# olsonanl/close_kmers

Measured on AMD Instinct MI355X. Metric: protein residues/s vs 1B-entry kmer image; 1/2/4/8 MI355X, higher is better.
Workload: dtype u64

## Files before the change

close_kmers_amd/csrc/kgx_internal.h:

```cpp
#ifndef KGX_INTERNAL_H
#define KGX_INTERNAL_H

#include <hip/hip_runtime.h>
#include <stdint.h>

#include "kgx.h"
#include "kgx_line_home.h"

namespace kgx {

constexpr int KMER = 8;
constexpr uint64_t CORE = 1280000000ULL;
constexpr uint64_t MAX_ENCODED = 25600000000ULL;
constexpr uint64_t EMPTY_KEY = MAX_ENCODED + 1;
constexpr int RUN_CAP = 40000 - 2;

constexpr int PROBE_WAVES = 4;
constexpr uint32_t HIT_PLANES = KGX_HIT_PLANES, HIT_PACKED16 = KGX_HIT_PACKED16;
constexpr int PROBE_BUCKET = 0;
constexpr int PROBE_KEY_FIRST = 1;
constexpr int PROBE_AUTO = -1;
constexpr int PROBE_LINE = 2;
constexpr int PROBE_LINE8 = 3;
constexpr int PROBE_J_DEFAULT = 2;
// ... 7 lines not shown

__host__ __device__ inline bool packable(const kgx_sig_kmer &e)
{
    return e.which_kmer > MAX_ENCODED ||
           (e.function_index >= -1 && e.function_index <= PACK_FI_MAX && e.otu_index >= -1 &&
            e.otu_index <= PACK_OTU_MAX);
}

__host__ __device__ inline packed_bucket pack_bucket(const kgx_sig_kmer &e)
{
    packed_bucket b;
    if (e.which_kmer > MAX_ENCODED) {
        b.lo = EMPTY_KEY;
        b.hi = 0;
        return b;
    }
    uint32_t wt;
    __builtin_memcpy(&wt, &e.function_wt, 4);
    const uint64_t fi = (uint64_t)(e.function_index + 1), otu = (uint64_t)(e.otu_index + 1);
    b.lo = e.which_kmer | (fi << 35) | ((otu & 0x1FFu) << 55);
    b.hi = (uint64_t)wt | ((uint64_t)e.avg_from_end << 32) | ((otu >> 9) << 48);
    return b;
}

__host__ __device__ inline kgx_sig_kmer unpack_bucket(const packed_bucket &b)
{
    kgx_sig_kmer e;
    e.which_kmer = b.lo & PACK_KEY_MASK;
    e.otu_index = (int32_t)(((b.lo >> 55) & 0x1FFu) | (((b.hi >> 48) & 0xFFFu) << 9)) - 1;
    e.avg_from_end = (uint16_t)(b.hi >> 32);
    e.pad = 0;
    e.function_index = (int32_t)((b.lo >> 35) & 0xFFFFFu) - 1;
    const uint32_t wt = (uint32_t)b.hi;
    __builtin_memcpy(&e.function_wt, &wt, 4);
    if (e.which_kmer > MAX_ENCODED) {
        e.otu_index = 0;
        e.avg_from_end = 0;
        e.function_index = 0;
        e.function_wt = 0.0f;
    }
    return e;
}

__host__ __device__ inline uint64_t filter_hash(uint64_t key)
{
    uint64_t h = key * 0x9E3779B97F4A7C15ull;
    return h ^ (h >> 29);
}
__host__ __device__ inline uint64_t filter_word(uint64_t h, uint32_t log2_words)
{
    return log2_words ? h >> (64 - log2_words) : 0;
}
__host__ __device__ inline uint64_t filter_bits(uint64_t h)
{
    return (1ull << (h & 63)) | (1ull << ((h >> 6) & 63));
}

inline uint64_t mod_magic(uint64_t n) { return n ? (~0ULL) / n : 0; }


size_t plan_workspace_bytes(uint32_t n_seq);
hipError_t launch_plan(const uint64_t *seq_off, uint32_t n_seq, uint64_t n_residues, uint64_t *wbase,
                       uint32_t *tile_seq, uint32_t tile_windows, void *workspace, uint32_t *status,
                       hipStream_t stream);
size_t plan_look_bytes(uint32_t n_seq);
hipError_t launch_plan_one(const uint64_t *seq_off, uint32_t n_seq, uint64_t n_residues, uint64_t *wbase,
                           uint32_t *tile_seq, uint32_t tile_windows, uint64_t max_tiles, uint32_t *status,
                           hipStream_t stream);
hipError_t launch_plan_fused(const uint64_t *seq_off, uint32_t n_seq, uint64_t n_residues, uint64_t *wbase,
                             uint32_t *tile_seq, uint32_t tile_windows, uint64_t max_tiles, void *look,
                             uint32_t *status, hipStream_t stream);

struct ProbeTable {
    const void *buckets;
    uint64_t num_sigs;
    uint32_t home;
    uint64_t magic() const { return mod_magic(num_sigs >> home_shift_of(home)); }
};
hipError_t launch_probe(const uint8_t *residues, uint64_t n_residues, const uint64_t *seq_off,
                        const uint64_t *wbase, const uint32_t *tile_seq, uint32_t n_seq,
                        uint64_t max_tiles, const ProbeTable &t, int layout,
                        const uint64_t *filter, uint32_t filter_log2_words,
                        uint4 *hot, uint4 *cold, uint64_t *hit_mask, int probe_j, int variant,
                        uint32_t lds_kb, uint32_t max_blocks, hipStream_t stream, uint32_t nt_stores = 0);
hipError_t launch_probe_dna(const uint8_t *bases, uint64_t n_bases, const uint64_t *anchor, const uint64_t *wbase,
                            const uint32_t *tile_seq, uint32_t n_seq, uint64_t max_tiles, const ProbeTable &t,
                            uint4 *hot, uint64_t *hit_mask, int probe_j, uint32_t max_blocks,
                            hipStream_t stream);

hipError_t launch_pack(const kgx_sig_kmer *table, packed_bucket *packed, uint64_t n,
                       uint32_t *not_packable, hipStream_t stream);
hipError_t launch_unpack(const packed_bucket *packed, kgx_sig_kmer *out, uint64_t n,
                         hipStream_t stream);
hipError_t launch_filter_build(const void *table, int layout, uint64_t num_sigs, uint64_t *filter,
                               uint32_t log2_words, hipStream_t stream);

enum { SCORE_HYBRID = 0, SCORE_WAVE = 1, SCORE_LANE = 2, SCORE_WAVE_ONLY = 3  };
constexpr uint32_t LONG_SEQ = 2048;
hipError_t launch_score(uint32_t n_seq, uint64_t n_residues, const uint64_t *wbase, const uint32_t *tile_seq,
                        uint64_t max_tiles, const uint64_t *hit_mask, uint32_t tile_windows, uint4 *hot,
                        kgx_call *calls, void *ranges, uint32_t *hit_count, uint32_t *call_count,
                        kgx_params params, uint32_t want, uint32_t hit_format, int variant, uint32_t wave_tiles,
                        const uint32_t *plan_status, hipStream_t stream);
hipError_t launch_best_calls(uint32_t n_seq, const kgx_call *calls, const uint64_t *start, const uint32_t *count,
                             kgx_call *ws, kgx_best_call *out, hipStream_t stream);
hipError_t launch_otus(uint32_t n_seq, const uint64_t *wbase, const uint64_t *hit_mask, uint32_t tile_windows,
                       const uint4 *hot, const uint4 *cold, int32_t *ws, kgx_otu *otus, uint32_t *otu_count,
                       uint32_t hit_format, hipStream_t stream);

constexpr uint32_t SMALL_GATHER_SEQ = 256;
constexpr uint32_t SMALL_COLLECT_BEST_SEQ = 8192;
constexpr uint32_t SMALL_GATHER_BLOCKS = 64;
hipError_t launch_small_gather(uint32_t n, const uint64_t *wbase, const uint64_t *hit_mask, uint32_t tile_windows,
                               const uint32_t *hit_count, const uint32_t *call_count, const uint4 *hot,
                               const uint4 *cold, const kgx_call *calls, const uint32_t *otu_count,
                               const kgx_otu *otus, kgx_hit *hits_out, kgx_call *calls_out, kgx_otu *otus_out,
                               uint64_t *h0, uint64_t *h1, uint64_t *h2, const uint32_t *status,
                               const kgx_best_call *best, kgx_best_call *best_host, uint32_t *status_host,
                               uint64_t *nwin_host, uint32_t *done_host, uint32_t token, uint32_t *blocks_done,
                               uint32_t hit_format, hipStream_t stream);
hipError_t launch_gather(uint32_t n_seq, const uint64_t *wbase, const uint64_t *hit_mask,
                         uint32_t tile_windows, const uint32_t *call_count, const uint4 *hot, const uint4 *cold,
                         const kgx_call *calls, const uint64_t *hit_dense_off,
                         const uint64_t *call_dense_off, kgx_hit *hits_out, kgx_call *calls_out,
                         uint32_t seq_base, uint32_t hit_format, const uint32_t *otu_count, const kgx_otu *otus,
                         const uint64_t *otu_dense_off, kgx_otu *otus_out, hipStream_t stream,
                         uint4 *hits16_out = nullptr,
                         uint32_t *hits12_out = nullptr);
size_t count_scan_workspace_bytes(uint32_t n);
hipError_t launch_count_scan(uint32_t n, const uint32_t *c0, const uint32_t *c1, const uint32_t *c2, uint64_t *o0,
                             uint64_t *o1, uint64_t *o2, void *workspace, hipStream_t stream);
constexpr int SMALL_PIECES = 5;
struct SmallPieces {
    uint4 *dst[SMALL_PIECES];
    const uint4 *src[SMALL_PIECES];
    uint64_t end16[SMALL_PIECES];
};
hipError_t launch_small_upload(const SmallPieces &pc, hipStream_t stream);
hipError_t launch_small_collect(uint32_t n, const uint32_t *c0, const uint32_t *c1, const uint32_t *c2, uint64_t *o0,
                                uint64_t *o1, uint64_t *o2, uint64_t *h0, uint64_t *h1, uint64_t *h2,
                                const uint32_t *status, const uint64_t *wbase, const kgx_best_call *best,
                                kgx_best_call *best_host, uint32_t *status_host, uint64_t *nwin_host,
                                hipStream_t stream);
hipError_t launch_small_collect_best(uint32_t n, const uint32_t *c0, const uint32_t *c1, const uint32_t *c2,
                                     uint64_t *o0, uint64_t *o1, uint64_t *o2, uint64_t *h0, uint64_t *h1,
                                     uint64_t *h2, const uint32_t *status, const uint64_t *wbase,
                                     const kgx_call *calls, const uint32_t *call_count, kgx_call *ws,
                                     kgx_best_call *best, kgx_best_call *best_host, uint32_t *status_host,
                                     uint64_t *nwin_host, hipStream_t stream);
hipError_t launch_copy_counted(void *dst, const void *src, const uint64_t *count, uint64_t cap,
                               uint32_t elem_bytes, int blocks, hipStream_t stream);
hipError_t launch_nul_scan(const uint8_t *d, uint64_t skip, uint64_t n, uint32_t *flag_mapped, hipStream_t stream);

hipError_t launch_copy_to_host(void *dst_mapped, const void *src, uint64_t bytes, int blocks, hipStream_t stream);
struct CopySpans {
    static constexpr int kMax = 8;
    void *dst[kMax];
    const void *src[kMax];
    uint64_t n[kMax];
    bool v16[kMax];
    int count = 0;
    void add(void *d, const void *s, uint64_t bytes)
    {
        if (bytes == 0)
            return;
        if (count == kMax) {
            count = kMax + 1;
            return;
        }
        dst[count] = d;
// ... 65 lines not shown
```

close_kmers_amd/csrc/kgx_probe.hip:

```cpp
#include <algorithm>

#include "kgx_device.h"

namespace kgx {

__device__ __forceinline__ uint3 load_residues(const uint8_t *residues, uint64_t bm, uint64_t n, uint64_t abo)
{
    uint32_t d[3] = {0, 0, 0};
    for (int b = 0; b < 12; b++)
        if (abo + b >= bm && abo + b < bm + n)
            d[b >> 2] |= (uint32_t)residues[abo + b - bm] << (8 * (b & 3));
    return make_uint3(d[0], d[1], d[2]);
}

constexpr int MODE_BUCKET = 0, MODE_KEY_FIRST = 1, MODE_PACKED = 2, MODE_PACKED_KEY_FIRST = 3;

typedef unsigned int u32x4_t __attribute__((ext_vector_type(4)));
template <bool NT> __device__ __forceinline__ uint4 load_record(const uint4 *p)
{
    if (NT) {
        const u32x4_t v = __builtin_nontemporal_load(reinterpret_cast<const u32x4_t *>(p));
        return make_uint4(v.x, v.y, v.z, v.w);
    }
    return *p;
// ... 260 lines not shown
                rec[j].x = m ? pv[j].x : rec[j].x;
                rec[j].y = m ? pv[j].y : rec[j].y;
                rec[j].z = m ? pv[j].z : rec[j].z;
                rec[j].w = m ? pv[j].w : rec[j].w;
            }
            if ((KEY_FIRST || MODE == MODE_PACKED_KEY_FIRST) && m) {
                if (KEY_FIRST)
                    rec[j] = *reinterpret_cast<const uint4 *>(
                        reinterpret_cast<const char *>(table + slot[j]) + 8);
                if (MODE == MODE_PACKED_KEY_FIRST) {
                    const uint64_t hi = packed_w[2 * slot[j] + 1];
                    rec[j] = make_uint4(pv[j].x, pv[j].y, (uint32_t)hi, (uint32_t)(hi >> 32));
                }
            }
            hit[j] = hit[j] || m;
            pend[j] = pend[j] && !m && !stop;
            slot[j] = pend[j] ? (slot[j] + 1 == num_sigs ? 0 : slot[j] + 1) : slot[j];
            more = more || pend[j];
        }
        if (!__any(more))
            break;
    }

    store_tile_hits<J, PACKED>(hit, key, rec, pos, sq, g0, W, lane, hot, cold, hit_mask);
}

__device__ __forceinline__ void probe_slice_aligned(const uint4 *__restrict__ packed, uint32_t n_lines, uint64_t key,
                                                    bool ok, uint32_t home_line, uint32_t q, uint32_t c, uint4 *rec,
                                                    uint8_t *hitf)
{
    constexpr uint32_t G = 4, NQ = 64 / G;
    constexpr uint32_t KEY_HI = (uint32_t)(PACK_KEY_MASK >> 32);
    constexpr uint32_t MAX_HI = (uint32_t)(MAX_ENCODED >> 32), MAX_LO = (uint32_t)MAX_ENCODED;
    static_assert(KEY_HI == 7u && (MARK_BITS_W & KEY_HI) == 0, "key bits 32-34 beside the mark bit");
    const uint32_t own = (uint32_t)(key >> 32) | (uint32_t)ok << 3 | line_mark(key) << 4;
    uint32_t klo[G], kw[G], ln[G];
    uint32_t live = 0;
#pragma unroll
    for (int i = 0; i < (int)G; i++) {
        const int owner = (int)(NQ * i + q);
        klo[i] = (uint32_t)__shfl((int)(uint32_t)key, owner);
        ln[i] = (uint32_t)__shfl((int)home_line, owner);
        const uint32_t o = (uint32_t)__shfl((int)own, owner);
        live |= (o >> 3 & 1u) << i;
        const uint32_t g = o >> 4;
        kw[i] = (o & KEY_HI) | (c == mark_record(g) ? 1u << mark_bit_w(g) : 0u);
    }
    const uint32_t cbit = 1u << c, upto = (2u << c) - 1u;
    constexpr uint32_t MARKED = 1u << G;
    const uint32_t max_lines = n_lines + 2;
    for (uint32_t round = 0;; round++) {
        uint4 d[G];
#pragma unroll
        for (int i = 0; i < (int)G; i++)
            if (live >> i & 1u)
                d[i] = packed[(uint64_t)ln[i] * G + c];
        uint32_t hitm = 0;
#pragma unroll
        for (int i = 0; i < (int)G; i++) {
            const uint32_t kh = d[i].y & KEY_HI;
            const uint32_t diff = (d[i].x ^ klo[i]) | ((d[i].y ^ kw[i]) & KEY_HI);
            const bool ends = diff == 0 || kh > MAX_HI || (kh == MAX_HI && d[i].x > MAX_LO);
            uint32_t w = (ends ? cbit : 0u) | ((d[i].w & kw[i]) >= 1u << 28 ? MARKED : 0u);
            w = live >> i & 1u ? w : 0u;
            w |= (uint32_t)xor_lane((int32_t)w, 1);
            w |= (uint32_t)xor_lane((int32_t)w, 2);
            hitm |= diff == 0 && (w & upto) == cbit ? 1u << i : 0u;
            live = (w & (2u * MARKED - 1)) == MARKED ? live : live & ~(1u << i);
            ln[i] = ln[i] + 1 == n_lines ? 0 : ln[i] + 1;
        }
#pragma unroll
        for (int i = 0; i < (int)G; i++)
            if (hitm >> i & 1u) {
                rec[NQ * i + q] = d[i];
                hitf[NQ * i + q] = 1;
            }
        if (round + 1 >= max_lines)
            live = 0;
        if (!__any(live != 0))
            break;
    }
}

template <int J, int G, bool DNA, bool MARKS, bool TWINS>
__global__ __launch_bounds__(256) void probe_line_kernel(
    const uint8_t *__restrict__ residues, uint64_t n_residues, const uint64_t *__restrict__ seq_off,
    const uint64_t *__restrict__ wbase, const uint32_t *__restrict__ tile_seq, uint32_t n_seq,
    const uint4 *__restrict__ packed, uint64_t num_sigs, uint64_t magic, uint32_t home, uint4 *__restrict__ hot,
    uint4 *__restrict__ cold, uint64_t *__restrict__ hit_mask, uint32_t nt)
{
    constexpr uint32_t T = 64 * J;
    constexpr uint32_t NQ = 64 / G;
    __shared__ uint8_t code_tab[256];
    __shared__ uint8_t cod_tab[DNA ? 68 : 1];
    __shared__ uint4 lds_rec[PROBE_WAVES][T];
    __shared__ uint8_t lds_hit[PROBE_WAVES][T];
    if (DNA) {
        const uint32_t b = threadIdx.x | 0x20u;
        const bool base = b == 'a' || b == 'c' || b == 'g' || b == 't' || b == 'u';
        code_tab[threadIdx.x] = base ? (uint8_t)(((b >> 1) ^ (b >> 2)) & 3u) : (uint8_t)0x40;
        if (threadIdx.x < 65)
            cod_tab[threadIdx.x] = threadIdx.x < 64 ? (uint8_t)residue_code((uint8_t)code11_aa(threadIdx.x)) : 20;
    } else {
        code_tab[threadIdx.x] = (uint8_t)residue_code(threadIdx.x);
    }
    __syncthreads();

    const uint32_t wave = __builtin_amdgcn_readfirstlane(threadIdx.x >> 6);
    const uint32_t lane = lane_id();
    const uint64_t W = wbase[n_seq];
    for (uint64_t tile = (uint64_t)blockIdx.x * PROBE_WAVES + wave; tile * T < W;
         tile += (uint64_t)gridDim.x * PROBE_WAVES) {
    const uint64_t g0 = tile * T;

    uint64_t key[J];
    uint32_t pos[J], sq[J];
    bool ok[J];
    const uint32_t q = lane / G, c = lane % G;
    static_assert(!MARKS || G == 4, "the index's lines are 4 records");
    static_assert(!TWINS || MARKS, "twin records come with marks only");
    if constexpr (MARKS) {
        uint32_t a7[J], b7[J];
        if (DNA)
            encode_tile_dna<J>(residues, n_residues, seq_off, wbase, tile_seq[tile], W, g0, lane, code_tab,
                               cod_tab, key, ok, pos, sq, a7, b7);
        else
            encode_tile<J>(residues, n_residues, seq_off, wbase, tile_seq[tile], W, g0, lane, code_tab, key, ok,
                           pos, sq, a7, b7);
        const uint32_t n_lines = (uint32_t)(num_sigs / G);
        uint32_t home_line[J];
#pragma unroll
        for (int j = 0; j < J; j++) {
            if (TWINS)
                home_line[j] = ok[j] ? (uint32_t)pair_home(a7[j], b7[j], lane, n_lines, magic) : 0;
            else
                home_line[j] = ok[j] ? (uint32_t)line_home_7mers(a7[j], b7[j], n_lines, magic, home_mode_of(home)) : 0;
            lds_hit[wave][64 * j + lane] = 0;
        }
#pragma unroll
        for (int j = 0; j < J; j++)
            probe_slice_aligned(packed, n_lines, key[j], ok[j], home_line[j], q, c, &lds_rec[wave][64 * j],
                                &lds_hit[wave][64 * j]);
    } else {
    if (DNA)
        encode_tile_dna<J>(residues, n_residues, seq_off, wbase, tile_seq[tile], W, g0, lane, code_tab, cod_tab,
                           key, ok, pos, sq);
    else
        encode_tile<J>(residues, n_residues, seq_off, wbase, tile_seq[tile], W, g0, lane, code_tab, key, ok,
                       pos, sq);
    uint64_t first[J];
#pragma unroll
    for (int j = 0; j < J; j++) {
        first[j] = ok[j] ? home_bucket(key[j], num_sigs, magic, home) : 0;
        lds_hit[wave][64 * j + lane] = 0;
    }

    const uint64_t max_lines = num_sigs / G + 2;
#pragma unroll
    for (int j = 0; j < J; j++) {
    uint64_t K[G], cur[G];
    uint32_t live = 0;
    const uint32_t own = (uint32_t)ok[j];
#pragma unroll
    for (int i = 0; i < G; i++) {
        const uint32_t owner = NQ * i + q;
        K[i] = __shfl(key[j], (int)owner);
        cur[i] = __shfl(first[j], (int)owner);
        const uint32_t o = (uint32_t)__shfl((int)own, (int)owner);
        live |= (o & 1u) << i;
    }
    for (uint64_t round = 0;; round++) {
        uint4 d[G];
#pragma unroll
        for (int i = 0; i < G; i++) {
            const uint64_t line = cur[i] - cur[i] % G;
            if ((live >> i & 1u) && line + c < num_sigs)
                d[i] = packed[line + c];
        }
        bool more = false;
#pragma unroll
        for (int i = 0; i < G; i++) {
            const bool act = live >> i & 1u;
            const uint64_t line = cur[i] - cur[i] % G;
            const uint64_t b = line + c;
            const uint64_t kb = ((uint64_t)d[i].y << 32 | d[i].x) & PACK_KEY_MASK;
            const bool valid = act && b < num_sigs && b >= cur[i];
            const uint64_t mm = __ballot(valid && kb == K[i]);
            const uint64_t me = __ballot(valid && kb > MAX_ENCODED);
            const uint32_t gm = (uint32_t)(mm >> (G * q)) & ((1u << G) - 1);
            const uint32_t ge = (uint32_t)(me >> (G * q)) & ((1u << G) - 1);
            if (act) {
                const uint32_t ev = gm | ge;
                if (ev) {
                    const uint32_t first = __builtin_ctz(ev);
                    if (c == first && (gm >> first & 1u)) {
                        const uint32_t w = 64 * j + NQ * i + q;
                        lds_rec[wave][w] = d[i];
                        lds_hit[wave][w] = 1;
                    }
                    live &= ~(1u << i);
                } else if (round + 1 >= max_lines) {
                    live &= ~(1u << i);
                } else {
                    cur[i] = line + G >= num_sigs ? 0 : line + G;
                    more = true;
                }
            }
        }
        if (!__any(more))
            break;
    }
    }
    }
    __builtin_amdgcn_fence(__ATOMIC_RELEASE, "wavefront");
    __builtin_amdgcn_wave_barrier();
    __builtin_amdgcn_fence(__ATOMIC_ACQUIRE, "wavefront");

    bool hit[J];
    uint4 pv[J];
#pragma unroll
    for (int j = 0; j < J; j++) {
        hit[j] = lds_hit[wave][64 * j + lane] != 0;
        pv[j] = hit[j] ? lds_rec[wave][64 * j + lane] : make_uint4(0, 0, 0, 0);
    }
    store_tile_hits<J, true>(hit, key, pv, pos, sq, g0, W, lane, hot, cold, hit_mask, nt != 0);
    }
}

template <int J, int G, bool DNA = false>
static void launch_probe_line(dim3 grid, hipStream_t stream, const uint8_t *residues, uint64_t n_residues,
                              const uint64_t *seq_off, const uint64_t *wbase, const uint32_t *tile_seq,
                              uint32_t n_seq, const ProbeTable &t, uint4 *hot, uint4 *cold, uint64_t *hit_mask,
                              uint32_t dyn_lds, uint32_t nt = 0)
{
    auto *kernel = probe_line_kernel<J, G, DNA, false, false>;
    if constexpr (G == 4)
        if (line_index_aligned(t.num_sigs, t.home))
            kernel = home_twins_of(t.home) ? probe_line_kernel<J, G, DNA, true, true>
                                           : probe_line_kernel<J, G, DNA, true, false>;
    hipLaunchKernelGGL(kernel, grid, dim3(64 * PROBE_WAVES), dyn_lds, stream, residues, n_residues, seq_off, wbase,
                       tile_seq, n_seq, static_cast<const uint4 *>(t.buckets), t.num_sigs, t.magic(), t.home, hot,
                       cold, hit_mask, nt);
}

template <int J, int MODE>
static void launch_probe_m(dim3 grid, hipStream_t stream, const uint8_t *residues, uint64_t n_residues,
                           const uint64_t *seq_off, const uint64_t *wbase, const uint32_t *tile_seq,
                           uint32_t n_seq, const ProbeTable &t, const uint64_t *filter, uint32_t filter_log2,
                           uint4 *hot, uint4 *cold, uint64_t *hit_mask)
{
    if (filter)
        hipLaunchKernelGGL((probe_kernel<J, MODE, true>), grid, dim3(64 * PROBE_WAVES), 0, stream, residues,
                           n_residues, seq_off, wbase, tile_seq, n_seq, t.buckets, t.num_sigs, t.magic(), t.home,
                           filter, filter_log2, hot, cold, hit_mask);
    else
        hipLaunchKernelGGL((probe_kernel<J, MODE, false>), grid, dim3(64 * PROBE_WAVES), 0, stream, residues,
                           n_residues, seq_off, wbase, tile_seq, n_seq, t.buckets, t.num_sigs, t.magic(), t.home,
                           filter, filter_log2, hot, cold, hit_mask);
}

template <int J>
static void launch_probe_j(dim3 grid, hipStream_t stream, int mode, const uint8_t *residues,
                           uint64_t n_residues, const uint64_t *seq_off, const uint64_t *wbase,
                           const uint32_t *tile_seq, uint32_t n_seq, const ProbeTable &t,
                           const uint64_t *filter, uint32_t filter_log2, uint4 *hot, uint4 *cold,
                           uint64_t *hit_mask)
{
#define KGX_PROBE_M(M)                                                                               \
    launch_probe_m<J, M>(grid, stream, residues, n_residues, seq_off, wbase, tile_seq, n_seq, t,     \
                         filter, filter_log2, hot, cold, hit_mask)
    if (mode == MODE_PACKED_KEY_FIRST)
        KGX_PROBE_M(MODE_PACKED_KEY_FIRST);
    else if (mode == MODE_PACKED)
        KGX_PROBE_M(MODE_PACKED);
    else if (mode == MODE_KEY_FIRST)
        KGX_PROBE_M(MODE_KEY_FIRST);
    else
        KGX_PROBE_M(MODE_BUCKET);
#undef KGX_PROBE_M
}

hipError_t launch_probe(const uint8_t *residues, uint64_t n_residues, const uint64_t *seq_off,
                        const uint64_t *wbase, const uint32_t *tile_seq, uint32_t n_seq,
                        uint64_t max_tiles, const ProbeTable &t, int layout,
                        const uint64_t *filter, uint32_t filter_log2,
                        uint4 *hot, uint4 *cold, uint64_t *hit_mask, int probe_j, int variant,
                        uint32_t lds_kb, uint32_t max_blocks, hipStream_t stream, uint32_t nt)
{
    if (max_tiles == 0)
        return hipSuccess;
    if (t.home && layout != KGX_LAYOUT_PACKED16)
        return hipErrorInvalidValue;
    const uint32_t dyn_lds = lds_kb * 1024u > 9216u ? lds_kb * 1024u - 9216u : 0u;
    const dim3 grid((uint32_t)((max_tiles + PROBE_WAVES - 1) / PROBE_WAVES));
    const dim3 lgrid(max_blocks ? std::min<uint32_t>(grid.x, max_blocks) : grid.x);
    if (variant == PROBE_AUTO && layout == KGX_LAYOUT_PACKED16 && !filter)
        variant = PROBE_LINE;
    if ((variant == PROBE_LINE || variant == PROBE_LINE8) && layout == KGX_LAYOUT_PACKED16 && !filter) {
#define KGX_LINE(JJ, GG)                                                                             \
    launch_probe_line<JJ, GG>(lgrid, stream, residues, n_residues, seq_off, wbase, tile_seq, n_seq, t,  \
                              hot, cold, hit_mask, dyn_lds, nt);                                     \
    return hipGetLastError()
        const int key = probe_j * 10 + (variant == PROBE_LINE8 ? 8 : 4);
        switch (key) {
        case 14: KGX_LINE(1, 4);
        case 24: KGX_LINE(2, 4);
        case 34: KGX_LINE(3, 4);
        case 44: KGX_LINE(4, 4);
        case 18: KGX_LINE(1, 8);
        case 28: KGX_LINE(2, 8);
        default: break;
        }
#undef KGX_LINE
    }
    const bool kf = variant == PROBE_AUTO ? layout != KGX_LAYOUT_PACKED16 : variant == PROBE_KEY_FIRST;
    const int mode = layout == KGX_LAYOUT_PACKED16 ? (kf ? MODE_PACKED_KEY_FIRST : MODE_PACKED)
                                                   : (kf ? MODE_KEY_FIRST : MODE_BUCKET);
#define KGX_PROBE_J(JJ)                                                                              \
    launch_probe_j<JJ>(grid, stream, mode, residues, n_residues, seq_off, wbase, tile_seq, n_seq,   \
                       t, filter, filter_log2, hot, cold, hit_mask)
    switch (probe_j) {
    case 1: KGX_PROBE_J(1); break;
    case 2: KGX_PROBE_J(2); break;
    case 3: KGX_PROBE_J(3); break;
    case 4: KGX_PROBE_J(4); break;
    case 5: KGX_PROBE_J(5); break;
    case 8: KGX_PROBE_J(8); break;
    default: return hipErrorInvalidValue;
    }
#undef KGX_PROBE_J
    return hipGetLastError();
}

hipError_t launch_probe_dna(const uint8_t *bases, uint64_t n_bases, const uint64_t *anchor, const uint64_t *wbase,
                            const uint32_t *tile_seq, uint32_t n_seq, uint64_t max_tiles, const ProbeTable &t,
                            uint4 *hot, uint64_t *hit_mask, int probe_j, uint32_t max_blocks,
                            hipStream_t stream)
{
    if (max_tiles == 0)
        return hipSuccess;
    const uint32_t tiles_grid = (uint32_t)((max_tiles + PROBE_WAVES - 1) / PROBE_WAVES);
    const dim3 grid(max_blocks ? std::min<uint32_t>(tiles_grid, max_blocks) : tiles_grid);
#define KGX_DNA(JJ)                                                                                  \
    launch_probe_line<JJ, 4, true>(grid, stream, bases, n_bases, anchor, wbase, tile_seq, n_seq, t,  \
                                   hot, nullptr, hit_mask, 0);                                       \
    return hipGetLastError()
    switch (probe_j) {
    case 1: KGX_DNA(1);
    case 2: KGX_DNA(2);
    case 3: KGX_DNA(3);
    case 4: KGX_DNA(4);
    default: return hipErrorInvalidValue;
    }
#undef KGX_DNA
}

}
```

close_kmers_amd/csrc/kgx_rt.h:

```cpp
#ifndef KGX_RT_H
#define KGX_RT_H

#include <hip/hip_runtime.h>

#include <algorithm>
#include <atomic>
#include <chrono>
#include <condition_variable>
#include <cstdio>
#include <cstdlib>
#include <cstring>
#include <deque>
#include <functional>
#include <memory>
#include <mutex>
#include <string>
#include <thread>
#include <vector>

#include "kgx_internal.h"
#include "kgx_options.h"

namespace kgx {

// ... 271 lines not shown
    explicit operator bool() const { return records != nullptr; }
    uint32_t home_word() const { return kgx::home_word(2u, home, marks, twins); }
};

}

struct kgx_image {
    int device = 0;
    uint64_t num_sigs = 0;
    int layout = KGX_LAYOUT_AOS24;
    kgx_sig_kmer *d_table = nullptr;
    kgx::packed_bucket *d_packed = nullptr;
    kgx::LineIndex lines;
    uint64_t *d_filter = nullptr;
    uint32_t filter_log2_words = 0;
    std::mutex probe_mu;
    hipEvent_t last_probe = nullptr;
    hipStream_t probe_stream = nullptr;
    std::mutex svc_mu;
    std::atomic<kgx::SvcState *> svc{nullptr};
    struct alignas(64) SvcUsers {
        std::atomic<uint32_t> n{0};
    };
    SvcUsers svc_users[32];
    uint32_t svc_slots = 32, svc_idle_us = 1000, svc_life_us = 1000;
    bool svc_configured = false;
    const void *resident() const
    {
        return layout == KGX_LAYOUT_PACKED16 ? static_cast<const void *>(d_packed) : d_table;
    }
    uint64_t resident_bytes() const
    {
        return num_sigs * (layout == KGX_LAYOUT_PACKED16 ? sizeof(kgx::packed_bucket) : sizeof(kgx_sig_kmer));
    }
    kgx::ProbeTable probe_table() const
    {
        return lines ? kgx::ProbeTable{lines.records, 4 * lines.n_lines, lines.home_word()} : reference_table();
    }
    kgx::ProbeTable reference_table() const { return kgx::ProbeTable{resident(), num_sigs, 0u}; }
};

struct kgx_ctx {
    kgx_image *img = nullptr;
    hipStream_t stream = nullptr;
    bool own_stream = false;
    hipEvent_t probe_done = nullptr;
    hipEvent_t probe_ready = nullptr;
    hipStream_t score_stream = nullptr;
    hipEvent_t score_gate = nullptr;
    kgx::DevBuf residues, offsets, wbase, tile_seq, hit_mask, hits, calls, hit_count, call_count,
        dense_hoff, dense_coff, dense_hits, dense_calls, plan_ws, ranges;
    kgx::DevBuf plan_status;
    kgx::DevBuf plan_look;
    kgx::PinnedVec<uint32_t> h_plan_status;
    uint32_t n_seq = 0;
    uint64_t n_residues = 0;
    uint64_t max_tiles = 0;
    uint32_t tile_windows = 64u * kgx::PROBE_J_DEFAULT;
    uint64_t hit_slots = 0;
    const uint64_t *d_off = nullptr;
    bool have_hits = false;
    uint32_t hit_format = kgx::HIT_PLANES;
    bool have_best = false;
    bool defer_best = false;
    kgx::DevBuf best, best_ws, bc_calls, bc_start, bc_count;
    kgx::PinnedVec<kgx_best_call> h_best;
    kgx::DevBuf fq_bases, fq_roff, fq_nfrag, fq_fbase, fq_tmp, fq_res, fq_off, fq_read, fq_frame, fq_start,
        fq_anchor, fq_nres;
    kgx::DevBuf fq_look;
    kgx::PinnedVec<uint64_t> h_fq_tot;
    kgx::FqPending fq_pend;
    struct {
        bool active = false;
        uint32_t n_reads = 0;
        uint64_t n_bases = 0;
    } fq_up;
    kgx::PinnedVec<uint64_t> h_fq_roff;
    kgx::DevBuf fqc_flag, fqc_reads, fqc_nsel, fqc_nfrag, fqc_ncall, fqc_fo, fqc_co, fqc_fc, fqc_len, fqc_coff,
        fqc_calls;
    kgx::PinnedVec<uint32_t> h_fqc_n, h_fqc_reads, h_fqc_fc, h_fqc_len;
    kgx::PinnedVec<uint64_t> h_fqc_tot, h_fqc_fo, h_fqc_coff;
    kgx::PinnedVec<kgx_call> h_fqc_calls;
    kgx::CtxOptions opt;
    std::vector<uint64_t> h_hoff, h_coff, h_ooff;
    kgx::PinnedVec<kgx_hit> h_hits;
    kgx::PinnedVec<kgx_call> h_calls;
    kgx::PinnedVec<kgx_otu> h_otus;
    kgx::PinnedVec<uint32_t> h_ocount;
    kgx::DevBuf otu_ws, otus, otu_count, dense_ooff, dense_otus;
    bool have_otus = false;
    kgx::PinnedVec<uint32_t> h_hcount, h_ccount;
    kgx::PinnedVec<char> h_res;
    kgx_ctx *twin = nullptr;
    kgx::PinnedVec<uint64_t> h_off_stage, h_dense_hoff, h_dense_coff, h_dense_ooff, h_nwin;
    std::unique_ptr<kgx::HostPool> pool;
    std::unique_ptr<kgx::HostPool> stage_pool;
    kgx::PinnedVec<uint4> h_hits16;
    kgx::PinnedVec<uint64_t> h_mask;
    std::vector<uint64_t> h_wstart;
    std::vector<hipEvent_t> chunk_done;
    std::vector<hipEvent_t> chunk_counts;
    std::vector<hipEvent_t> chunk_gathered;
    hipStream_t copy_stream = nullptr;
    hipStream_t up_stream = nullptr;
    kgx::DevBuf up_res, up_off;
    kgx::DevBuf dense_mask, dense_best;
    double rate_hits = 0.35, rate_calls = 0.05, rate_otus = 0.05;
    uint64_t stream_fallbacks = 0;
    bool one_pass_pinned = false;
    uint64_t pinned_batches = 0, nul_reruns = 0;
    uint32_t counts_enqueued = 0;
    kgx::PinnedVec<uint32_t> h_nul;
    std::vector<hipEvent_t> chunk_h2d;
    kgx::DevBuf dense_counts, cscan_ws;
    kgx::PinnedVec<uint32_t> h_counts;
    kgx::PinnedVec<uint32_t> h_hits12;
    kgx::PinnedVec<char> h_res_all;
    kgx::PinnedVec<uint64_t> h_off_all;
    kgx::PinnedVec<uint4> h_small;
    kgx::PinnedVec<uint32_t> h_done;
    kgx::DevBuf small_blocks_done;
    uint64_t fused_batches = 0, small_batches = 0;
    kgx::PinnedVec<uint64_t> h_fwb;
    kgx::PinnedVec<kgx_hit> h_fhits;
    kgx::PinnedVec<kgx_call> h_fcalls;
    kgx::PinnedVec<uint32_t> h_fcounts, h_fdone;
    kgx::PinnedVec<uint64_t> h_fdbg;
    uint32_t small_token = 0;
    kgx::PinnedVec<kgx_call> h_calls_region;
    kgx::PinnedVec<kgx_otu> h_otus_region;
    int compact_out = 0;
    struct CompactSeg {
        uint32_t s0, s1, words;
        uint64_t hit_begin, rec_at, mask_at;
    };
    std::vector<CompactSeg> compact_segs;
    std::vector<kgx_hit_chunk> compact_chunks;
    std::vector<hipEvent_t> prof_ev;
    std::vector<hipEvent_t> prof_done;
    kgx_host_profile last_profile{};
    std::unique_ptr<kgx::RollupScratch> rollup;
};

namespace kgx {
static_assert(CtxOptions{}.probe_variant == PROBE_AUTO && CtxOptions{}.probe_j == PROBE_J_DEFAULT,
              "kgx_options.h spells these two defaults as numbers");
inline void drop_line_index(kgx_image *img)
{
    if (img->lines)
        (void)hipFree(img->lines.records);
    img->lines = LineIndex{};
}
inline bool ctx_lines(const kgx_ctx *c) { return c->img->lines && c->opt.line_index; }
inline ProbeTable ctx_probe_table(const kgx_ctx *c)
{
    return ctx_lines(c) ? c->img->probe_table() : c->img->reference_table();
}
inline void fill_result(kgx_ctx *c, uint32_t n_seq, bool need_hits, bool want_best, uint64_t nwin, kgx_result *out)
{
    out->best = want_best ? c->h_best.data() : nullptr;
    out->n_seq = n_seq;
    out->hit_offsets = c->h_hoff.data();
    out->hits = need_hits ? c->h_hits.data() : nullptr;
    out->call_offsets = c->h_coff.data();
    out->calls = c->h_calls.data();
    out->otu_offsets = c->h_ooff.data();
// ... 28 lines not shown
```

close_kmers_amd/csrc/kgx_runtime.cpp:

```cpp
#include <hip/hip_runtime.h>
#include <sched.h>

#include <algorithm>
#include <cerrno>
#include <ctime>
#include <chrono>
#include <cstdio>
#include <cstdlib>
#include <cstring>
#include <map>
#include <stdexcept>
#include <string>
#include <atomic>
#include <fcntl.h>
#include <mutex>
#include <sys/stat.h>
#include <thread>
#include <unistd.h>
#include <vector>

#include "kgx_rt.h"

using namespace kgx;

// ... 771 lines not shown
    return KGX_OK;
}

int kgx_image_set_layout(kgx_image *img, int layout)
{
    if (!img)
        return fail(KGX_EINVAL, "null image");
    const auto hold = svc_shutdown_hold(img);
    if (layout == KGX_LAYOUT_PACKED16)
        return image_pack(img);
    if (layout == KGX_LAYOUT_AOS24) {
        if (img->lines) {
            HIP_TRY(hipSetDevice(img->device));
            HIP_TRY(hipDeviceSynchronize());
            drop_line_index(img);
        }
        return image_unpack(img);
    }
    return fail(KGX_EINVAL, "unknown layout " + std::to_string(layout));
}

static int image_read(const kgx_image *img, uint64_t first, uint64_t count, kgx_sig_kmer *dst)
{
    HIP_TRY(hipSetDevice(img->device));
    if (img->layout == KGX_LAYOUT_AOS24) {
        HIP_TRY(hipMemcpy(dst, img->d_table + first, count * sizeof(kgx_sig_kmer), hipMemcpyDeviceToHost));
        return KGX_OK;
    }
    const uint64_t slice = 1ull << 24;
    kgx_sig_kmer *tmp = nullptr;
    HIP_TRY(hipMalloc(&tmp, std::max<uint64_t>(1, std::min(slice, count)) * sizeof(kgx_sig_kmer)));
    hipError_t e = hipSuccess;
    for (uint64_t b = 0; b < count && e == hipSuccess; b += slice) {
        const uint64_t m = std::min(slice, count - b);
        e = launch_unpack(img->d_packed + first + b, tmp, m, nullptr);
        if (e == hipSuccess)
            e = hipMemcpy(dst + b, tmp, m * sizeof(kgx_sig_kmer), hipMemcpyDeviceToHost);
    }
    (void)hipFree(tmp);
    if (e != hipSuccess)
        return fail(KGX_EDEVICE, std::string("download: ") + hipGetErrorString(e));
    return KGX_OK;
}

int kgx_image_download(const kgx_image *img, void *dst, uint64_t nbytes)
{
    if (!img || !dst || nbytes != img->num_sigs * sizeof(kgx_sig_kmer))
        return fail(KGX_EINVAL, "bad download buffer");
    return image_read(img, 0, img->num_sigs, static_cast<kgx_sig_kmer *>(dst));
}

int kgx_image_save(const kgx_image *img, const char *dir)
{
    if (!img || !dir)
        return fail(KGX_EINVAL, "null argument");
    const std::string path = std::string(dir) + "/kmer.table.mem_map";
    FILE *f = std::fopen(path.c_str(), "wb");
    if (!f)
        return fail(KGX_EIO, "could not open " + path + " for writing: " + std::strerror(errno));
    const kgx_image_header h{img->num_sigs, sizeof(kgx_sig_kmer), 1};
    bool ok = std::fwrite(&h, sizeof(h), 1, f) == 1;
    const uint64_t chunk = 1ull << 25;
    std::vector<kgx_sig_kmer> buf(std::min(chunk, std::max<uint64_t>(img->num_sigs, 1)));
    for (uint64_t b = 0; ok && b < img->num_sigs; b += chunk) {
        const uint64_t m = std::min(chunk, img->num_sigs - b);
        int rc = image_read(img, b, m, buf.data());
        if (rc) {
            std::fclose(f);
            return rc;
        }
        ok = std::fwrite(buf.data(), sizeof(kgx_sig_kmer), m, f) == m;
    }
    if (std::fclose(f) != 0)
        ok = false;
    return ok ? KGX_OK : fail(KGX_EIO, "short write to " + path);
}


int kgx_ctx_create(kgx_image *img, kgx_ctx **out)
{
    if (!img || !out)
        return fail(KGX_EINVAL, "null argument");
    HIP_TRY(hipSetDevice(img->device));
    kgx_ctx *c = new kgx_ctx;
    c->img = img;
    hipError_t e = hipStreamCreateWithFlags(&c->stream, hipStreamNonBlocking);
    if (e != hipSuccess) {
        delete c;
        return fail(KGX_EDEVICE, std::string("stream: ") + hipGetErrorString(e));
    }
    c->own_stream = true;
    if (const char *sb = std::getenv("KGX_SMALL_BATCH"))
        c->opt.small_batch = std::min<int64_t>(1 << 24, std::max<int64_t>(0, std::atoll(sb)));
    e = hipEventCreateWithFlags(&c->probe_done, hipEventDisableTiming);
    if (e != hipSuccess) {
        (void)hipStreamDestroy(c->stream);
        delete c;
        return fail(KGX_EDEVICE, std::string("event: ") + hipGetErrorString(e));
    }
    *out = c;
    return KGX_OK;
}

int kgx_ctx_destroy(kgx_ctx *c)
{
    if (!c)
        return KGX_OK;
    (void)hipSetDevice(c->img->device);
    if (c->twin)
        kgx_ctx_destroy(c->twin);
    (void)hipStreamSynchronize(c->stream);
    for (DevBuf *b : {&c->residues, &c->offsets, &c->wbase, &c->tile_seq, &c->hit_mask,
                      &c->hits, &c->calls, &c->hit_count, &c->call_count, &c->dense_hoff,
                      &c->dense_coff, &c->dense_hits, &c->dense_calls, &c->plan_ws, &c->ranges})
        b->release();
    {
        std::lock_guard<std::mutex> lock(c->img->probe_mu);
        if (c->img->last_probe == c->probe_done)
            c->img->last_probe = nullptr;
    }
    (void)hipEventDestroy(c->probe_done);
    if (c->probe_ready)
        (void)hipEventDestroy(c->probe_ready);
    if (c->score_gate)
        (void)hipEventDestroy(c->score_gate);
    c->pool.reset();
    c->stage_pool.reset();
    for (hipEvent_t e : c->chunk_done)
        (void)hipEventDestroy(e);
    for (hipEvent_t e : c->chunk_counts)
        (void)hipEventDestroy(e);
    for (hipEvent_t e : c->chunk_gathered)
        (void)hipEventDestroy(e);
    for (hipEvent_t e : c->chunk_h2d)
        (void)hipEventDestroy(e);
    for (hipEvent_t e : c->prof_ev)
        (void)hipEventDestroy(e);
    for (hipEvent_t e : c->prof_done)
        (void)hipEventDestroy(e);
    if (c->copy_stream) {
        (void)hipStreamSynchronize(c->copy_stream);
        (void)hipStreamDestroy(c->copy_stream);
    }
    if (c->up_stream) {
        (void)hipStreamSynchronize(c->up_stream);
        (void)hipStreamDestroy(c->up_stream);
    }
    if (c->own_stream)
        (void)hipStreamDestroy(c->stream);
    delete c;
    return KGX_OK;
}

void *kgx_ctx_stream(kgx_ctx *c) { return c ? (void *)c->stream : nullptr; }

int kgx_ctx_set_stream(kgx_ctx *c, void *stream)
{
    if (!c)
        return fail(KGX_EINVAL, "null ctx");
    if (stream) {
        if (c->own_stream)
            (void)hipStreamDestroy(c->stream);
        c->stream = (hipStream_t)stream;
        c->own_stream = false;
    } else if (!c->own_stream) {
        HIP_TRY(hipStreamCreateWithFlags(&c->stream, hipStreamNonBlocking));
        c->own_stream = true;
    }
// ... 98 lines not shown
    c->have_otus = false;
    return KGX_OK;
}

}

namespace {

uint32_t probe_max_blocks(const kgx_ctx *c)
{
    if (!c->opt.probe_persist)
        return 0;
    int cus = 0;
    if (hipDeviceGetAttribute(&cus, hipDeviceAttributeMultiprocessorCount, c->img->device) != hipSuccess || cus <= 0)
        cus = 256;
    return (uint32_t)c->opt.probe_persist * (uint32_t)cus;
}

template <class Launch>
int probe_chained(kgx_ctx *c, Launch launch)
{
    HIP_TRY(hipSetDevice(c->img->device));
    if (c->img->num_sigs >= (1ull << 40))
        return fail(KGX_ERANGE, "image too large");
    kgx_image *img = c->img;
    std::unique_lock<std::mutex> lock(img->probe_mu, std::defer_lock);
    if (c->opt.probe_serialize && c->opt.probe_stream) {
        lock.lock();
        if (!img->probe_stream)
            HIP_TRY(hipStreamCreateWithFlags(&img->probe_stream, hipStreamNonBlocking));
        if (!c->probe_ready)
            HIP_TRY(hipEventCreateWithFlags(&c->probe_ready, hipEventDisableTiming));
        HIP_TRY(hipEventRecord(c->probe_ready, c->stream));
        HIP_TRY(hipStreamWaitEvent(img->probe_stream, c->probe_ready, 0));
        hipStream_t own = c->stream;
        c->stream = img->probe_stream;
        const hipError_t le = launch();
        c->stream = own;
        HIP_TRY(le);
        HIP_TRY(hipEventRecord(c->probe_done, img->probe_stream));
        HIP_TRY(hipStreamWaitEvent(c->stream, c->probe_done, 0));
        img->last_probe = c->probe_done;
    } else {
        if (c->opt.probe_serialize) {
            lock.lock();
            if (img->last_probe && img->last_probe != c->probe_done)
                HIP_TRY(hipStreamWaitEvent(c->stream, img->last_probe, 0));
        }
        HIP_TRY(launch());
        if (c->opt.probe_serialize) {
            HIP_TRY(hipEventRecord(c->probe_done, c->stream));
            img->last_probe = c->probe_done;
        }
    }
    c->hit_format = c->img->layout == KGX_LAYOUT_PACKED16 ? HIT_PACKED16 : HIT_PLANES;
    c->have_hits = true;
    return KGX_OK;
}

}

namespace kgx {

bool probe_takes_dna(const kgx_ctx *c)
{
    return c->img->layout == KGX_LAYOUT_PACKED16 && !(c->opt.probe_filter && c->img->d_filter) &&
           (c->opt.probe_variant == PROBE_AUTO || c->opt.probe_variant == PROBE_LINE) && c->opt.probe_j >= 1 && c->opt.probe_j <= 4;
}

int stage_probe_dna(kgx_ctx *c, const uint8_t *bases, uint64_t n_bases, const uint64_t *anchors,
                    const uint64_t *d_off)
{
    if ((!anchors || !bases) && c->n_seq)
        return fail(KGX_EINVAL, "fq probe: anchors or bases missing");
    if (d_off != c->d_off)
        return fail(KGX_EINVAL, "fq probe: offsets differ from the plan");
    if (!probe_takes_dna(c) || (int)(c->tile_windows / 64) != c->opt.probe_j)
        return fail(KGX_EINVAL, "fq probe: fragments without residues need the line probe on a PACKED16 image "
                                "(set fq_residues 1 for other probes)");
    return probe_chained(c, [&] {
        return launch_probe_dna(bases, n_bases, anchors, c->wbase.as<uint64_t>(), c->tile_seq.as<uint32_t>(),
                                c->n_seq, c->max_tiles, ctx_probe_table(c),
                                c->hits.as<uint4>(), c->hit_mask.as<uint64_t>(), (int)(c->tile_windows / 64),
                                probe_max_blocks(c), c->stream);
    });
}

}

extern "C" {

int kgx_stage_probe(kgx_ctx *c, const uint8_t *d_res, const uint64_t *d_off)
{
    if (!c || (!d_res && c->n_residues) || d_off != c->d_off)
        return fail(KGX_EINVAL, "probe: residues missing or offsets differ from the plan");
    return probe_chained(c, [&] {
        return launch_probe(d_res, c->n_residues, d_off, c->wbase.as<uint64_t>(), c->tile_seq.as<uint32_t>(),
                            c->n_seq, c->max_tiles, ctx_probe_table(c), c->img->layout,
                            c->opt.probe_filter ? c->img->d_filter : nullptr, c->img->filter_log2_words,
                            c->hits.as<uint4>(), c->hits.as<uint4>() + c->hit_slots, c->hit_mask.as<uint64_t>(),
                            (int)(c->tile_windows / 64), c->opt.probe_variant, (uint32_t)c->opt.probe_lds_kb,
                            probe_max_blocks(c), c->stream, (uint32_t)c->opt.probe_nt);
    });
}



int kgx_stage_score(kgx_ctx *c, const kgx_params *params, uint32_t want)
{
    if (!c)
        return fail(KGX_EINVAL, "null ctx");
    kgx_params p;
    if (params)
        p = *params;
    else
        kgx_params_default(&p);
    HIP_TRY(hipSetDevice(c->img->device));
    const bool best = (want & KGX_WANT_BEST) != 0;
    HIP_TRY(launch_score(c->n_seq, c->n_residues, c->wbase.as<uint64_t>(), c->tile_seq.as<uint32_t>(), c->max_tiles,
                         c->hit_mask.as<uint64_t>(), c->tile_windows, c->hits.as<uint4>(), c->calls.as<kgx_call>(),
                         c->ranges.p, c->hit_count.as<uint32_t>(), c->call_count.as<uint32_t>(), p,
                         want | (best ? KGX_WANT_CALLS : 0u), c->hit_format, c->opt.score_variant,
                         (uint32_t)c->opt.score_wave_tiles, c->plan_status.as<uint32_t>(), c->stream));
    c->have_best = false;
    c->have_otus = false;
    if (want & KGX_WANT_OTU) {
        HIP_TRY(c->otu_ws.reserve(std::max<uint64_t>(c->hit_slots, 1) * sizeof(int32_t)));
        HIP_TRY(c->otus.reserve(std::max<uint64_t>(c->hit_slots, 1) * sizeof(kgx_otu)));
        HIP_TRY(c->otu_count.reserve(std::max<uint64_t>(c->n_seq, 1) * sizeof(uint32_t)));
        HIP_TRY(launch_otus(c->n_seq, c->wbase.as<uint64_t>(), c->hit_mask.as<uint64_t>(), c->tile_windows,
                            c->hits.as<uint4>(), c->hits.as<uint4>() + c->hit_slots, c->otu_ws.as<int32_t>(),
                            c->otus.as<kgx_otu>(), c->otu_count.as<uint32_t>(), c->hit_format, c->stream));
        c->have_otus = true;
    }
    if (best) {
        HIP_TRY(c->best.reserve(std::max<uint64_t>(c->n_seq, 1) * sizeof(kgx_best_call)));
        HIP_TRY(c->best_ws.reserve(c->hit_slots * sizeof(kgx_call)));
        if (!c->defer_best)
            HIP_TRY(launch_best_calls(c->n_seq, c->calls.as<kgx_call>(), c->wbase.as<uint64_t>(),
                                      c->call_count.as<uint32_t>(), c->best_ws.as<kgx_call>(),
                                      c->best.as<kgx_best_call>(), c->stream));
        c->have_best = true;
    }
    return KGX_OK;
}

int kgx_find_best_calls(kgx_ctx *c, const kgx_call *calls, const uint64_t *call_offsets, uint32_t n_seq,
                        kgx_best_call *out)
{
    if (!c || (n_seq && (!call_offsets || !out)))
        return fail(KGX_EINVAL, "null argument");
    if (n_seq == 0)
        return KGX_OK;
    const uint64_t c0 = call_offsets[0], n = call_offsets[n_seq] - c0;
    if (n && !calls)
        return fail(KGX_EINVAL, "null calls");
    std::vector<uint64_t> start(n_seq);
    std::vector<uint32_t> count(n_seq);
    for (uint32_t s = 0; s < n_seq; s++) {
        if (call_offsets[s + 1] < call_offsets[s])
            return fail(KGX_EINVAL, "call_offsets not monotone");
        start[s] = call_offsets[s] - c0;
        count[s] = (uint32_t)(call_offsets[s + 1] - call_offsets[s]);
    }
    HIP_TRY(hipSetDevice(c->img->device));
    HIP_TRY(c->bc_calls.reserve(std::max<uint64_t>(n, 1) * sizeof(kgx_call)));
    HIP_TRY(c->best_ws.reserve(std::max<uint64_t>(n, 1) * sizeof(kgx_call)));
    HIP_TRY(c->bc_start.reserve(n_seq * sizeof(uint64_t)));
    HIP_TRY(c->bc_count.reserve(n_seq * sizeof(uint32_t)));
    HIP_TRY(c->best.reserve(n_seq * sizeof(kgx_best_call)));
    c->have_best = false;
    if (n)
        HIP_TRY(hipMemcpyAsync(c->bc_calls.p, calls + c0, n * sizeof(kgx_call), hipMemcpyHostToDevice, c->stream));
    HIP_TRY(hipMemcpyAsync(c->bc_start.p, start.data(), n_seq * sizeof(uint64_t), hipMemcpyHostToDevice, c->stream));
    HIP_TRY(hipMemcpyAsync(c->bc_count.p, count.data(), n_seq * sizeof(uint32_t), hipMemcpyHostToDevice, c->stream));
    HIP_TRY(launch_best_calls(n_seq, c->bc_calls.as<kgx_call>(), c->bc_start.as<uint64_t>(),
                              c->bc_count.as<uint32_t>(), c->best_ws.as<kgx_call>(), c->best.as<kgx_best_call>(),
                              c->stream));
    HIP_TRY(hipMemcpyAsync(out, c->best.p, n_seq * sizeof(kgx_best_call), hipMemcpyDeviceToHost, c->stream));
    HIP_TRY(hipStreamSynchronize(c->stream));
    return KGX_OK;
}

int kgx_device_result_get(kgx_ctx *c, kgx_device_result *out)
{
// ... 360 lines not shown
```

Baseline: 58.94 billion.

## Defer multi-round line probes into a compacted per-wave list

Adds a deferred probe mode for the aligned G=4 line kernel. It does the first line round for every window slice, then compacts the windows still open into a per-wave LDS list. It then runs the later rounds over that list, 16 keys at a time, so lanes stay busy instead of idling while a few slices chain through many lines. This costs extra LDS (open list and stashed key state), a wave barrier, and more bookkeeping. The mode is on by default, and the environment variable KGX_PROBE_DEFER can switch it off.

```diff
diff --git a/close_kmers_amd/csrc/kgx_internal.h b/close_kmers_amd/csrc/kgx_internal.h
--- a/close_kmers_amd/csrc/kgx_internal.h
+++ b/close_kmers_amd/csrc/kgx_internal.h
@@ -113,10 +113,11 @@
                         uint64_t max_tiles, const ProbeTable &t, int layout,
                         const uint64_t *filter, uint32_t filter_log2_words,
                         uint4 *hot, uint4 *cold, uint64_t *hit_mask, int probe_j, int variant,
-                        uint32_t lds_kb, uint32_t max_blocks, hipStream_t stream, uint32_t nt_stores = 0);
+                        uint32_t lds_kb, uint32_t max_blocks, bool defer, hipStream_t stream,
+                        uint32_t nt_stores = 0);
 hipError_t launch_probe_dna(const uint8_t *bases, uint64_t n_bases, const uint64_t *anchor, const uint64_t *wbase,
                             const uint32_t *tile_seq, uint32_t n_seq, uint64_t max_tiles, const ProbeTable &t,
-                            uint4 *hot, uint64_t *hit_mask, int probe_j, uint32_t max_blocks,
+                            uint4 *hot, uint64_t *hit_mask, int probe_j, uint32_t max_blocks, bool defer,
                             hipStream_t stream);
 
 hipError_t launch_pack(const kgx_sig_kmer *table, packed_bucket *packed, uint64_t n,
diff --git a/close_kmers_amd/csrc/kgx_probe.hip b/close_kmers_amd/csrc/kgx_probe.hip
--- a/close_kmers_amd/csrc/kgx_probe.hip
+++ b/close_kmers_amd/csrc/kgx_probe.hip
@@ -366,7 +366,100 @@
     }
 }
 
-template <int J, int G, bool DNA, bool MARKS, bool TWINS>
+__device__ __forceinline__ uint32_t quad_line_word(const uint4 &d, uint32_t klo, uint32_t kw, bool open,
+                                                   uint32_t cbit, uint32_t &diff)
+{
+    constexpr uint32_t KEY_HI = (uint32_t)(PACK_KEY_MASK >> 32), MARKED = 1u << 4;
+    constexpr uint32_t MAX_HI = (uint32_t)(MAX_ENCODED >> 32), MAX_LO = (uint32_t)MAX_ENCODED;
+    const uint32_t kh = d.y & KEY_HI;
+    diff = (d.x ^ klo) | ((d.y ^ kw) & KEY_HI);
+    const bool ends = diff == 0 || kh > MAX_HI || (kh == MAX_HI && d.x > MAX_LO);
+    uint32_t w = (ends ? cbit : 0u) | ((d.w & kw) >= 1u << 28 ? MARKED : 0u);
+    w = open ? w : 0u;
+    w |= (uint32_t)xor_lane((int32_t)w, 1);
+    w |= (uint32_t)xor_lane((int32_t)w, 2);
+    return w;
+}
+
+__device__ __forceinline__ uint32_t probe_slice_round0(const uint4 *__restrict__ packed, uint64_t key, uint32_t own,
+                                                       uint32_t home_line, uint32_t q, uint32_t c, uint4 *rec,
+                                                       uint8_t *hitf)
+{
+    constexpr uint32_t G = 4, NQ = 64 / G, MARKED = 1u << G;
+    constexpr uint32_t KEY_HI = (uint32_t)(PACK_KEY_MASK >> 32);
+    uint32_t klo[G], kw[G], ln[G];
+    uint32_t live = 0;
+#pragma unroll
+    for (int i = 0; i < (int)G; i++) {
+        const int owner = (int)(NQ * i + q);
+        klo[i] = (uint32_t)__shfl((int)(uint32_t)key, owner);
+        ln[i] = (uint32_t)__shfl((int)home_line, owner);
+        const uint32_t o = (uint32_t)__shfl((int)own, owner);
+        live |= (o >> 3 & 1u) << i;
+        const uint32_t g = o >> 4;
+        kw[i] = (o & KEY_HI) | (c == mark_record(g) ? 1u << mark_bit_w(g) : 0u);
+    }
+    const uint32_t cbit = 1u << c, upto = (2u << c) - 1u;
+    uint4 d[G];
+#pragma unroll
+    for (int i = 0; i < (int)G; i++)
+        if (live >> i & 1u)
+            d[i] = packed[(uint64_t)ln[i] * G + c];
+    uint32_t hitm = 0;
+#pragma unroll
+    for (int i = 0; i < (int)G; i++) {
+        uint32_t diff;
+        const uint32_t w = quad_line_word(d[i], klo[i], kw[i], live >> i & 1u, cbit, diff);
+        hitm |= diff == 0 && (w & upto) == cbit ? 1u << i : 0u;
+        live = (w & (2u * MARKED - 1)) == MARKED ? live : live & ~(1u << i);
+    }
+#pragma unroll
+    for (int i = 0; i < (int)G; i++)
+        if (hitm >> i & 1u) {
+            rec[NQ * i + q] = d[i];
+            hitf[NQ * i + q] = 1;
+        }
+    return live;
+}
+
+__device__ __forceinline__ void probe_tile_deferred(const uint4 *__restrict__ packed, uint32_t n_lines,
+                                                    uint32_t n_open, const uint8_t *list, uint32_t q, uint32_t c,
+                                                    uint4 *rec, uint8_t *hitf)
+{
+    constexpr uint32_t G = 4, NQ = 64 / G, MARKED = 1u << G;
+    constexpr uint32_t KEY_HI = (uint32_t)(PACK_KEY_MASK >> 32);
+    const uint32_t cbit = 1u << c, upto = (2u << c) - 1u;
+    const uint32_t max_lines = n_lines + 2;
+    for (uint32_t p = 0; p < n_open; p += NQ) {
+        bool live = p + q < n_open;
+        uint32_t w = 0;
+        uint4 e = make_uint4(0, 0, 0, 0);
+        if (live) {
+            w = list[p + q];
+            e = rec[w];
+        }
+        const uint32_t klo = e.x, g = e.y >> 4;
+        const uint32_t kw = (e.y & KEY_HI) | (c == mark_record(g) ? 1u << mark_bit_w(g) : 0u);
+        uint32_t ln = e.z;
+        for (uint32_t round = 1;; round++) {
+            uint4 d;
+            if (live)
+                d = packed[(uint64_t)ln * G + c];
+            uint32_t diff;
+            const uint32_t lw = quad_line_word(d, klo, kw, live, cbit, diff);
+            if (diff == 0 && (lw & upto) == cbit) {
+                rec[w] = d;
+                hitf[w] = 1;
+            }
+            live = live && (lw & (2u * MARKED - 1)) == MARKED && round + 1 < max_lines;
+            ln = ln + 1 == n_lines ? 0 : ln + 1;
+            if (!__any(live))
+                break;
+        }
+    }
+}
+
+template <int J, int G, bool DNA, bool MARKS, bool TWINS, bool DEFER>
 __global__ __launch_bounds__(256) void probe_line_kernel(
     const uint8_t *__restrict__ residues, uint64_t n_residues, const uint64_t *__restrict__ seq_off,
     const uint64_t *__restrict__ wbase, const uint32_t *__restrict__ tile_seq, uint32_t n_seq,
@@ -379,6 +472,8 @@
     __shared__ uint8_t cod_tab[DNA ? 68 : 1];
     __shared__ uint4 lds_rec[PROBE_WAVES][T];
     __shared__ uint8_t lds_hit[PROBE_WAVES][T];
+    __shared__ uint8_t lds_open[PROBE_WAVES][DEFER ? T : 1];
+    static_assert(T <= 256, "a window slot is a byte of lds_open");
     if (DNA) {
         const uint32_t b = threadIdx.x | 0x20u;
         const bool base = b == 'a' || b == 'c' || b == 'g' || b == 't' || b == 'u';
@@ -421,10 +516,33 @@
                 home_line[j] = ok[j] ? (uint32_t)line_home_7mers(a7[j], b7[j], n_lines, magic, home_mode_of(home)) : 0;
             lds_hit[wave][64 * j + lane] = 0;
         }
+        if constexpr (DEFER) {
+            uint32_t n_open = 0;
+#pragma unroll
+            for (int j = 0; j < J; j++) {
+                const uint32_t own = (uint32_t)(key[j] >> 32) | (uint32_t)ok[j] << 3 | line_mark(key[j]) << 4;
+                const uint32_t live = probe_slice_round0(packed, key[j], own, home_line[j], q, c,
+                                                         &lds_rec[wave][64 * j], &lds_hit[wave][64 * j]);
+                const uint32_t of_quad = (uint32_t)__shfl((int)live, (int)(G * (lane % NQ)));
+                const bool open = of_quad >> (lane / NQ) & 1u;
+                const uint64_t m = __ballot(open);
+                if (open) {
+                    const uint32_t next = home_line[j] + 1 == n_lines ? 0 : home_line[j] + 1;
+                    lds_rec[wave][64 * j + lane] = make_uint4((uint32_t)key[j], own, next, 0);
+                    lds_open[wave][n_open + lanes_below(m)] = (uint8_t)(64 * j + lane);
+                }
+                n_open += (uint32_t)__popcll(m);
+            }
+            __builtin_amdgcn_fence(__ATOMIC_RELEASE, "wavefront");
+            __builtin_amdgcn_wave_barrier();
+            __builtin_amdgcn_fence(__ATOMIC_ACQUIRE, "wavefront");
+            probe_tile_deferred(packed, n_lines, n_open, lds_open[wave], q, c, lds_rec[wave], lds_hit[wave]);
+        } else {
 #pragma unroll
         for (int j = 0; j < J; j++)
             probe_slice_aligned(packed, n_lines, key[j], ok[j], home_line[j], q, c, &lds_rec[wave][64 * j],
                                 &lds_hit[wave][64 * j]);
+        }
     } else {
     if (DNA)
         encode_tile_dna<J>(residues, n_residues, seq_off, wbase, tile_seq[tile], W, g0, lane, code_tab, cod_tab,
@@ -515,13 +633,18 @@
 static void launch_probe_line(dim3 grid, hipStream_t stream, const uint8_t *residues, uint64_t n_residues,
                               const uint64_t *seq_off, const uint64_t *wbase, const uint32_t *tile_seq,
                               uint32_t n_seq, const ProbeTable &t, uint4 *hot, uint4 *cold, uint64_t *hit_mask,
-                              uint32_t dyn_lds, uint32_t nt = 0)
-{
-    auto *kernel = probe_line_kernel<J, G, DNA, false, false>;
+                              uint32_t dyn_lds, bool defer, uint32_t nt = 0)
+{
+    auto *kernel = probe_line_kernel<J, G, DNA, false, false, false>;
     if constexpr (G == 4)
-        if (line_index_aligned(t.num_sigs, t.home))
-            kernel = home_twins_of(t.home) ? probe_line_kernel<J, G, DNA, true, true>
-                                           : probe_line_kernel<J, G, DNA, true, false>;
+        if (line_index_aligned(t.num_sigs, t.home)) {
+            if (defer)
+                kernel = home_twins_of(t.home) ? probe_line_kernel<J, G, DNA, true, true, true>
+                                               : probe_line_kernel<J, G, DNA, true, false, true>;
+            else
+                kernel = home_twins_of(t.home) ? probe_line_kernel<J, G, DNA, true, true, false>
+                                               : probe_line_kernel<J, G, DNA, true, false, false>;
+        }
     hipLaunchKernelGGL(kernel, grid, dim3(64 * PROBE_WAVES), dyn_lds, stream, residues, n_residues, seq_off, wbase,
                        tile_seq, n_seq, static_cast<const uint4 *>(t.buckets), t.num_sigs, t.magic(), t.home, hot,
                        cold, hit_mask, nt);
@@ -569,13 +692,14 @@
                         uint64_t max_tiles, const ProbeTable &t, int layout,
                         const uint64_t *filter, uint32_t filter_log2,
                         uint4 *hot, uint4 *cold, uint64_t *hit_mask, int probe_j, int variant,
-                        uint32_t lds_kb, uint32_t max_blocks, hipStream_t stream, uint32_t nt)
+                        uint32_t lds_kb, uint32_t max_blocks, bool defer, hipStream_t stream, uint32_t nt)
 {
     if (max_tiles == 0)
         return hipSuccess;
     if (t.home && layout != KGX_LAYOUT_PACKED16)
         return hipErrorInvalidValue;
-    const uint32_t dyn_lds = lds_kb * 1024u > 9216u ? lds_kb * 1024u - 9216u : 0u;
+    const uint32_t own_lds = defer ? 9728u : 9216u;
+    const uint32_t dyn_lds = lds_kb * 1024u > own_lds ? lds_kb * 1024u - own_lds : 0u;
     const dim3 grid((uint32_t)((max_tiles + PROBE_WAVES - 1) / PROBE_WAVES));
     const dim3 lgrid(max_blocks ? std::min<uint32_t>(grid.x, max_blocks) : grid.x);
     if (variant == PROBE_AUTO && layout == KGX_LAYOUT_PACKED16 && !filter)
@@ -583,7 +707,7 @@
     if ((variant == PROBE_LINE || variant == PROBE_LINE8) && layout == KGX_LAYOUT_PACKED16 && !filter) {
 #define KGX_LINE(JJ, GG)                                                                             \
     launch_probe_line<JJ, GG>(lgrid, stream, residues, n_residues, seq_off, wbase, tile_seq, n_seq, t,  \
-                              hot, cold, hit_mask, dyn_lds, nt);                                     \
+                              hot, cold, hit_mask, dyn_lds, defer, nt);                              \
     return hipGetLastError()
         const int key = probe_j * 10 + (variant == PROBE_LINE8 ? 8 : 4);
         switch (key) {
@@ -618,7 +742,7 @@
 
 hipError_t launch_probe_dna(const uint8_t *bases, uint64_t n_bases, const uint64_t *anchor, const uint64_t *wbase,
                             const uint32_t *tile_seq, uint32_t n_seq, uint64_t max_tiles, const ProbeTable &t,
-                            uint4 *hot, uint64_t *hit_mask, int probe_j, uint32_t max_blocks,
+                            uint4 *hot, uint64_t *hit_mask, int probe_j, uint32_t max_blocks, bool defer,
                             hipStream_t stream)
 {
     if (max_tiles == 0)
@@ -627,7 +751,7 @@
     const dim3 grid(max_blocks ? std::min<uint32_t>(tiles_grid, max_blocks) : tiles_grid);
 #define KGX_DNA(JJ)                                                                                  \
     launch_probe_line<JJ, 4, true>(grid, stream, bases, n_bases, anchor, wbase, tile_seq, n_seq, t,  \
-                                   hot, nullptr, hit_mask, 0);                                       \
+                                   hot, nullptr, hit_mask, 0, defer);                                \
     return hipGetLastError()
     switch (probe_j) {
     case 1: KGX_DNA(1);
diff --git a/close_kmers_amd/csrc/kgx_rt.h b/close_kmers_amd/csrc/kgx_rt.h
--- a/close_kmers_amd/csrc/kgx_rt.h
+++ b/close_kmers_amd/csrc/kgx_rt.h
@@ -377,6 +377,7 @@
     kgx::PinnedVec<uint64_t> h_fqc_tot, h_fqc_fo, h_fqc_coff;
     kgx::PinnedVec<kgx_call> h_fqc_calls;
     kgx::CtxOptions opt;
+    bool probe_defer = true;
     std::vector<uint64_t> h_hoff, h_coff, h_ooff;
     kgx::PinnedVec<kgx_hit> h_hits;
     kgx::PinnedVec<kgx_call> h_calls;
diff --git a/close_kmers_amd/csrc/kgx_runtime.cpp b/close_kmers_amd/csrc/kgx_runtime.cpp
--- a/close_kmers_amd/csrc/kgx_runtime.cpp
+++ b/close_kmers_amd/csrc/kgx_runtime.cpp
@@ -877,8 +877,15 @@
     if (!img || !out)
         return fail(KGX_EINVAL, "null argument");
     HIP_TRY(hipSetDevice(img->device));
+    bool probe_defer = true;
+    if (const char *pd = std::getenv("KGX_PROBE_DEFER"); pd && *pd) {
+        if (std::strcmp(pd, "0") && std::strcmp(pd, "1"))
+            return fail(KGX_EINVAL, std::string("KGX_PROBE_DEFER: 0 (rounds per slice) or 1 (deferred), not \"") + pd + "\"");
+        probe_defer = pd[0] == '1';
+    }
     kgx_ctx *c = new kgx_ctx;
     c->img = img;
+    c->probe_defer = probe_defer;
     hipError_t e = hipStreamCreateWithFlags(&c->stream, hipStreamNonBlocking);
     if (e != hipSuccess) {
         delete c;
@@ -1143,7 +1150,7 @@
         return launch_probe_dna(bases, n_bases, anchors, c->wbase.as<uint64_t>(), c->tile_seq.as<uint32_t>(),
                                 c->n_seq, c->max_tiles, ctx_probe_table(c),
                                 c->hits.as<uint4>(), c->hit_mask.as<uint64_t>(), (int)(c->tile_windows / 64),
-                                probe_max_blocks(c), c->stream);
+                                probe_max_blocks(c), c->probe_defer, c->stream);
     });
 }
 
@@ -1161,7 +1168,7 @@
                             c->opt.probe_filter ? c->img->d_filter : nullptr, c->img->filter_log2_words,
                             c->hits.as<uint4>(), c->hits.as<uint4>() + c->hit_slots, c->hit_mask.as<uint64_t>(),
                             (int)(c->tile_windows / 64), c->opt.probe_variant, (uint32_t)c->opt.probe_lds_kb,
-                            probe_max_blocks(c), c->stream, (uint32_t)c->opt.probe_nt);
+                            probe_max_blocks(c), c->probe_defer, c->stream, (uint32_t)c->opt.probe_nt);
     });
 }
 
```

After: 64.92 billion (median of 6 runs). 1.1x the previous value.
